# Xiugapurin/Etude

Hardware: AMD Instinct MI355X
Metric: audio-sec/s transcribed + decoder tokens/s, 3-min clip batch (higher is better)
Workload: dtype f16

## Files before the change

### etude_amd/_lib.py

```python
from __future__ import annotations

import ctypes as C
import os
from pathlib import Path

import torch

LIB_PATH = Path(os.environ["ETD_LIB_PATH"]) if os.environ.get("ETD_LIB_PATH") else Path(__file__).resolve().parent / "libetude_hip.so"

c_int_p = C.POINTER(C.c_int)
c_i32_p = C.POINTER(C.c_int32)
c_i64_p = C.POINTER(C.c_int64)
c_f32_p = C.POINTER(C.c_float)


class _SizedCfg(C.Structure):

    def __init__(self, *a, **k):
        super().__init__(*a, **k)
        self.struct_bytes = C.sizeof(type(self))


class ExtCfg(_SizedCfg):
    _fields_ = [("struct_bytes", C.c_int)] + [(n, C.c_int) for n in ("n_margin", "n_frame", "n_bin", "cnn_channel", "cnn_kernel", "hid_dim", "pf_dim",
# ... 80 lines not shown
class Job(C.Structure):
    _fields_ = [("x_ids", C.c_void_p), ("x_offsets", C.c_void_p), ("n_bars", C.c_int), ("attrs4", C.c_void_p), ("ready", C.c_void_p)]


class ScoreJob(C.Structure):
    _fields_ = [("x_ids", C.c_void_p), ("x_offsets", C.c_void_p), ("n_bars", C.c_int), ("attrs4", C.c_void_p),
                ("y_ids", C.c_void_p), ("y_offsets", C.c_void_p), ("n_y_bars", C.c_int)]


class SchedCfg(_SizedCfg):
    _fields_ = [("struct_bytes", C.c_int)] + [(n, C.c_int) for n in ("bar_bos_id", "bar_eos_id", "n_ctx_pairs", "max_position_embeddings", "max_output_tokens",
                                       "max_bar_token_limit")] + [("context_overlap_ratio", C.c_float)] + \
               [(n, C.c_int) for n in ("force_bar_tokens", "max_streams", "max_prefill_rows", "steps_per_poll")] + \
               [("temperature", C.c_float), ("top_p", C.c_float), ("seed", C.c_ulonglong), ("job_key_offset", C.c_int), ("job_key_stride", C.c_int)]


class TempoRegion(C.Structure):
    _fields_ = [("bpm", C.c_double), ("time_sig", C.c_int), ("start", C.c_double), ("downbeats", C.c_void_p), ("n_downbeats", C.c_int)]


class TokEvent(C.Structure):
    _fields_ = [("type", C.c_int32), ("value", C.c_int32)]


class Note(C.Structure):
    _fields_ = [("onset", C.c_double), ("offset", C.c_double), ("pitch", C.c_int32), ("velocity", C.c_int32)]


ABI_VERSION = 3

SIGNATURES = {
    "etd_version": (C.c_int, []),
    "etd_last_error": (C.c_char_p, []),
    "etd_build_id": (C.c_char_p, []),
    "etd_extractor_operand_type": (C.c_int, []),
    "etd_decoder_operand_type": (C.c_int, []),
    "etd_has_experiments": (C.c_int, []),
    "etd_prof_enable": (C.c_int, [C.c_int]),
    "etd_prof_reset": (C.c_int, []),
    "etd_prof_collect": (C.c_int, []),
    "etd_prof_count": (C.c_int, []),
    "etd_prof_entry": (C.c_int, [C.c_int, C.c_char_p, C.c_int, C.POINTER(C.c_double), C.POINTER(C.c_longlong),
                                 C.POINTER(C.c_double), C.POINTER(C.c_double)]),
    "etd_debug_boundary_cost": (C.c_int, [C.c_int, C.c_int, C.c_int, C.c_void_p, C.POINTER(C.c_double), C.POINTER(C.c_double)]),
    "etd_debug_linear": (C.c_int, [C.c_int, C.c_int, C.c_int, C.c_int, C.c_void_p, C.POINTER(C.c_double)]),
    "etd_debug_kernel_loop": (C.c_int, [C.c_int, C.c_int, C.c_void_p]),
    "etd_debug_g3_bounds": (C.c_int, [C.c_void_p, C.c_void_p, C.c_int, C.c_int, C.c_void_p, C.c_void_p, C.c_float, C.c_void_p, C.c_void_p]),
    "etd_debug_gemm3": (C.c_int, [C.c_void_p, C.c_int, C.c_int, C.c_void_p, C.c_void_p, C.c_int, C.c_float, C.c_int, C.c_void_p, C.c_void_p, C.c_void_p, C.c_void_p]),
    "etd_debug_gemm3_case": (C.c_int, [C.POINTER(G3Case), C.c_void_p]),
    "etd_debug_ln_rows_f32": (C.c_int, [C.c_void_p, C.c_int, C.c_int, C.c_void_p, C.c_void_p, C.c_void_p, C.c_void_p, C.c_float, C.c_void_p, C.c_void_p, C.c_void_p]),
    "etd_debug_g3_pack": (C.c_int, [C.c_void_p, C.c_int, C.c_int, C.c_void_p, C.c_longlong, C.POINTER(C.c_longlong), C.POINTER(C.c_int32)]),
    "etd_debug_attn3": (C.c_int, [C.c_void_p, C.c_void_p, C.c_void_p, C.c_void_p, C.c_int, C.c_int, C.c_int, C.c_int, C.c_float, C.c_float, C.c_float, C.c_int, C.c_void_p, C.c_void_p]),
    "etd_debug_empty_launch": (C.c_int, [C.c_int, C.c_int, C.c_int, C.c_void_p, C.c_void_p]),
    "etd_frontend_create": (C.c_int, [C.c_int, C.c_int, C.c_int, C.c_int, C.c_int, C.c_int, C.c_void_p, C.c_int, C.c_int,
                                      C.c_void_p, C.c_int, C.c_void_p, C.c_void_p, C.c_void_p, C.c_float, C.POINTER(C.c_void_p)]),
    "etd_frontend_destroy": (None, [C.c_void_p]),
    "etd_frontend_set_pad_mode": (C.c_int, [C.c_void_p, C.c_int]),
    "etd_rms_frames": (C.c_int, [C.c_void_p, C.c_longlong, C.c_int, C.c_int, C.c_void_p, C.c_longlong, C.c_void_p]),
    "etd_frontend_resampled_len": (C.c_longlong, [C.c_void_p, C.c_longlong]),
    "etd_frontend_num_frames": (C.c_longlong, [C.c_void_p, C.c_longlong]),
    "etd_frontend_run": (C.c_int, [C.c_void_p, C.c_void_p, C.c_int, C.c_longlong, C.c_void_p, C.c_void_p, C.c_longlong,
                                   C.POINTER(C.c_longlong), C.c_void_p]),
    "etd_extractor_create": (C.c_int, [C.POINTER(ExtCfg), C.POINTER(C.c_char_p), C.POINTER(C.c_void_p), c_i64_p, C.c_int,
                                       C.POINTER(C.c_void_p)]),
    "etd_extractor_destroy": (None, [C.c_void_p]),
    "etd_transcript": (C.c_int, [C.c_void_p, C.c_void_p, C.c_longlong] + [C.c_void_p] * 8 + [C.c_void_p]),
    "etd_transcript_windows": (C.c_int, [C.c_void_p, C.c_void_p, C.c_int] + [C.c_void_p] * 8 + [C.c_void_p]),
    "etd_extractor_debug_vel_logits": (C.c_int, [C.c_void_p, C.c_void_p]),
    "etd_extractor_debug_tap": (C.c_int, [C.c_void_p, C.c_int, C.c_void_p]),
    "etd_extractor_window_flops": (C.c_double, [C.c_void_p]),
    "etd_mpe2note": (C.c_int, [C.c_void_p, C.c_void_p, C.c_void_p, C.c_void_p, C.c_longlong, C.c_int, C.c_float, C.c_float,
                               C.c_float, C.c_int, C.c_int, C.c_int, C.POINTER(Note), C.c_longlong, C.POINTER(C.c_longlong)]),
    "etd_mpe2note_modes": (C.c_int, [C.c_void_p, C.c_void_p, C.c_void_p, C.c_void_p, C.c_longlong, C.c_int, C.c_float, C.c_float,
                                     C.c_float, C.c_int, C.c_int, C.c_int, C.c_int, C.c_int, C.POINTER(Note), C.c_longlong, C.POINTER(C.c_longlong)]),
    "etd_mpe2note_dev_create": (C.c_int, [C.c_int, C.POINTER(C.c_void_p)]),
    "etd_mpe2note_dev_destroy": (None, [C.c_void_p]),
    "etd_mpe2note_dev": (C.c_int, [C.c_void_p, C.c_void_p, C.c_void_p, C.c_void_p, C.c_void_p, C.c_longlong, C.c_float, C.c_float, C.c_float,
                                   C.c_int, C.c_int, C.c_int, C.POINTER(Note), C.c_longlong, C.POINTER(C.c_longlong), C.c_void_p]),
    "etd_mpe2note_dev_modes": (C.c_int, [C.c_void_p, C.c_void_p, C.c_void_p, C.c_void_p, C.c_void_p, C.c_longlong, C.c_float, C.c_float, C.c_float,
                                         C.c_int, C.c_int, C.c_int, C.c_int, C.c_int, C.POINTER(Note), C.c_longlong, C.POINTER(C.c_longlong), C.c_void_p]),
    "etd_tok_create": (C.c_int, [C.c_void_p, C.c_int, C.POINTER(C.c_void_p)]),
    "etd_tok_destroy": (None, [C.c_void_p]),
    "etd_tok_num_measures": (C.c_int, [C.c_void_p]),
    "etd_tok_measures": (C.c_int, [C.c_void_p, C.c_void_p, C.c_void_p, C.c_void_p, C.c_void_p]),
    "etd_tok_encode": (C.c_int, [C.c_void_p, C.c_void_p, C.c_longlong, C.c_int, C.c_void_p, C.c_longlong, C.POINTER(C.c_longlong)]),
    "etd_tok_split_bars": (C.c_int, [C.c_void_p, C.c_longlong, C.c_int, C.c_int, C.c_void_p, C.c_longlong, C.c_void_p, C.c_longlong,
                                     C.POINTER(C.c_longlong)]),
    "etd_tok_decode": (C.c_int, [C.c_void_p, C.c_void_p, C.c_longlong, C.c_void_p, C.c_longlong, C.c_void_p, C.c_longlong,
                                 C.POINTER(C.c_longlong)]),
    "etd_midi_write": (C.c_int, [C.c_void_p, C.c_longlong, C.c_char_p]),
    "etd_decoder_create": (C.c_int, [C.POINTER(DecCfg), C.POINTER(C.c_char_p), C.POINTER(C.c_void_p), c_i64_p, C.c_int,
                                     C.POINTER(C.c_void_p)]),
    "etd_decoder_destroy": (None, [C.c_void_p]),
    "etd_decoder_clone": (C.c_int, [C.c_void_p, C.POINTER(C.c_void_p)]),
    "etd_decoder_set_sampling": (C.c_int, [C.c_void_p, C.c_float, C.c_float, C.c_ulonglong, C.c_void_p]),
    "etd_decoder_set_keys": (C.c_int, [C.c_void_p, C.c_int, C.c_void_p, C.c_void_p]),
    "etd_decoder_begin_bar": (C.c_int, [C.c_void_p, C.c_int, C.c_void_p, C.c_void_p, C.c_void_p, C.c_int, C.c_void_p, C.c_int,
                                        C.c_int, C.c_void_p]),
    "etd_decoder_begin_bars": (C.c_int, [C.c_void_p, C.c_int] + [C.c_void_p] * 8 + [C.c_void_p]),
    "etd_decoder_step": (C.c_int, [C.c_void_p, C.c_void_p, C.c_int, C.c_int, C.c_void_p]),
    "etd_decoder_poll": (C.c_int, [C.c_void_p, C.c_void_p, C.c_int, C.c_void_p, C.c_void_p, C.c_void_p]),
    "etd_decoder_read_tokens": (C.c_int, [C.c_void_p, C.c_int, C.c_void_p, C.c_int, c_int_p, C.c_void_p]),
    "etd_decoder_read_many": (C.c_int, [C.c_void_p, C.c_int, C.c_void_p, C.c_void_p, C.c_int, C.c_void_p, C.c_void_p]),
    "etd_decoder_run_jobs": (C.c_int, [C.c_void_p, C.POINTER(SchedCfg), C.POINTER(Job), C.c_int, C.c_void_p, C.c_longlong, C.c_void_p,
                                       C.POINTER(C.c_longlong), C.c_void_p]),
    "etd_debug_assemble_prompt": (C.c_int, [C.POINTER(SchedCfg), C.c_int, C.c_void_p, C.c_void_p, C.c_void_p, C.c_void_p, C.c_void_p, C.c_void_p,
# ... 148 lines not shown
```

### etude_amd/csrc/dec_fused.hip

```cpp
#include "dec_epilogue.h"
#include "dec_kernels.h"
#include "prof.h"

#include <cstdlib>
#include <utility>
#define PM_SLOT_ELEMS (32 * 1024)

typedef const __attribute__((address_space(1))) void* pm_gptr_t;
typedef __attribute__((address_space(3))) void* pm_lptr_t;

template <int F> __device__ __forceinline__ void pm_rd(d16x8& b, unsigned addr) {
  asm volatile("ds_read_b128 %0, %1 offset:%2" : "=v"(b) : "v"(addr), "n"(F * 1024));
}
template <int F0> __device__ __forceinline__ void pm_rd4(d16x8 (&b)[4], unsigned addr) {
  pm_rd<F0>(b[0], addr); pm_rd<F0 + 1>(b[1], addr); pm_rd<F0 + 2>(b[2], addr); pm_rd<F0 + 3>(b[3], addr);
}
template <int N> __device__ __forceinline__ void pm_wait_lds() { asm volatile("s_waitcnt lgkmcnt(%0)" ::"n"(N) : "memory"); }
__device__ __forceinline__ void pm_mfma_v_a(f32x16& acc, const d16x8& af, const d16x8& bf) {
  asm volatile(ETD_MFMA16_DEC " %0, %1, %2, %0" : "+v"(acc) : "v"(af), "a"(bf));
}
template <int T, bool B_AGPR> __device__ __forceinline__ void pm_mfma_out(f32x16& acc, const d16x8& af, const d16x8& bf) {
  if constexpr (T < 8) {
    if constexpr (B_AGPR) asm volatile(ETD_MFMA16_DEC " %0, %1, %2, %0" : "+a"(acc) : "v"(af), "a"(bf));
    else                  asm volatile(ETD_MFMA16_DEC " %0, %1, %2, %0" : "+a"(acc) : "v"(af), "v"(bf));
  } else {
    if constexpr (B_AGPR) asm volatile(ETD_MFMA16_DEC " %0, %1, %2, %0" : "+v"(acc) : "v"(af), "a"(bf));
    else                  asm volatile(ETD_MFMA16_DEC " %0, %1, %2, %0" : "+v"(acc) : "v"(af), "v"(bf));
  }
}
struct PmNext { const d16* src; d16* dst; bool on; };
template <int I> __device__ __forceinline__ void pm_dma(const PmNext& n) {
  if (n.on) __builtin_amdgcn_global_load_lds((pm_gptr_t)(n.src + (I >> 2) * 2048), (pm_lptr_t)(n.dst + (I >> 2) * 2048), 16, (I & 3) * 1024, 0);
}
template <int J> struct PmMlpGroup { static constexpr int f0 = J < 8 ? 32 + 4 * J : 4 * (J - 8); };
template <int J, int JEND> __device__ __forceinline__ void pm_roll(d16x8 (&buf)[2][4], unsigned addr) {
  if constexpr (J + 1 < JEND) { pm_rd4<PmMlpGroup<J + 1>::f0>(buf[(J + 1) & 1], addr); pm_wait_lds<4>(); }
  else pm_wait_lds<0>();
}
template <int J> __device__ __forceinline__ void pm_gelu2(f32x16& acc1, const float* sbu, int kc, int h) {
#pragma unroll
  for (int e = 0; e < 2; ++e) {
    constexpr int dummy = 0; (void)dummy;
    const int i = 2 * J + e;
    acc1[i] = gelu_fast(acc1[i] + sbu[32 * kc + 8 * (i >> 2) + 4 * h + (i & 3)]);
  }
}
template <int J> __device__ __forceinline__ void pm_up_group0(d16x8 (&buf)[2][4], unsigned addr, f32x16& accn, const d16x8 (&xf)[32], const PmNext& nx) {
  pm_roll<J, 8>(buf, addr);
#pragma unroll
  for (int q = 0; q < 4; ++q) pm_mfma_v_a(accn, buf[J & 1][q], xf[4 * J + q]);
  pm_dma<2 * J>(nx); pm_dma<2 * J + 1>(nx);
  __builtin_amdgcn_sched_barrier(0);
}
template <int J, bool HALF> __device__ __forceinline__ void pm_down_group(d16x8 (&buf)[2][4], unsigned addr, f32x16 (&acc2)[16], const d16x8 (&hf)[2], const PmNext& nx) {
  pm_roll<J, 16>(buf, addr);
  constexpr int g = J - 8, t0 = 4 * (g & 3);
  pm_mfma_out<t0 + 0, false>(acc2[t0 + 0], buf[J & 1][0], hf[g >> 2]);
  pm_mfma_out<t0 + 1, false>(acc2[t0 + 1], buf[J & 1][1], hf[g >> 2]);
  pm_mfma_out<t0 + 2, false>(acc2[t0 + 2], buf[J & 1][2], hf[g >> 2]);
// ... 105 lines not shown
  if constexpr (ND >= 2) pm_dma<D0 + 1>(nx);
#undef PM_MFMA
#undef PM_PIN
  __builtin_amdgcn_sched_barrier(0);
}
template <int KS> __device__ __forceinline__ void pm_hidden_frag1(const f32x16& acc1, d16x8& hfk) {
  const d16x4 p0 = pack4d(acc1[8 * KS], acc1[8 * KS + 1], acc1[8 * KS + 2], acc1[8 * KS + 3]);
  const d16x4 p1 = pack4d(acc1[8 * KS + 4], acc1[8 * KS + 5], acc1[8 * KS + 6], acc1[8 * KS + 7]);
  const u32x2 v0 = __builtin_bit_cast(u32x2, p0), v1 = __builtin_bit_cast(u32x2, p1);
  const auto s0 = __builtin_amdgcn_permlane32_swap(v0[0], v1[0], false, false);
  const auto s1 = __builtin_amdgcn_permlane32_swap(v0[1], v1[1], false, false);
  const u32x4 o = {s0[0], s1[0], s0[1], s1[1]};
  hfk = __builtin_bit_cast(d16x8, o);
  asm volatile("s_nop 4" : "+v"(hfk) : : "memory");
}
#define PM_LOADX(dst, ptr, S) asm volatile("global_load_dwordx4 %0, %1, off offset:%2" : "=a"(dst) : "v"(ptr), "n"(32 * (S)) : "memory")
template <bool AOL>
__device__ __forceinline__ void pm_chunk(d16x8 (&buf)[2][4], unsigned sa, f32x16& prev, f32x16& cur, f32x16 (&acc2)[16], d16x8 (&xf)[32], d16x8 (&hf)[2],
                                         unsigned bias_prev, unsigned bias_cur, const PmNext& nx, const d16* ao, long long ao_off) {
  const d16* ap = nullptr;
  if constexpr (AOL) { ap = ao + ao_off; asm volatile("" : "+v"(ap)); }
#define PM_AOL(G) do { if constexpr (AOL) { PM_LOADX(xf[4 * (G)], ap, 4 * (G)); PM_LOADX(xf[4 * (G) + 1], ap, 4 * (G) + 1); PM_LOADX(xf[4 * (G) + 2], ap, 4 * (G) + 2); PM_LOADX(xf[4 * (G) + 3], ap, 4 * (G) + 3); } } while (0)
  pm_rd4<PmMlpGroup<0>::f0>(buf[0], sa);
  pm_group<0, 4, 0, 2>(buf, sa, cur, acc2, xf, hf[0], prev, bias_prev, nx);
  pm_group<1, 5, 2, 2>(buf, sa, cur, acc2, xf, hf[0], prev, bias_prev, nx);
  pm_group<2, 6, 4, 1>(buf, sa, cur, acc2, xf, hf[0], prev, bias_prev, nx);
  pm_group<3, 7, 5, 1>(buf, sa, cur, acc2, xf, hf[0], prev, bias_prev, nx);
  pm_group<4, 8, 6, 2>(buf, sa, cur, acc2, xf, hf[0], prev, bias_prev, nx);
  pm_group<5, 9, 8, 2>(buf, sa, cur, acc2, xf, hf[0], prev, bias_prev, nx);
  pm_group<6, 10, 10, 1>(buf, sa, cur, acc2, xf, hf[0], prev, bias_prev, nx);
  pm_group<7, 11, 11, 1>(buf, sa, cur, acc2, xf, hf[0], prev, bias_prev, nx);
  pm_hidden_frag1<0>(prev, hf[0]);
  pm_group<8, 12, 12, 1>(buf, sa, cur, acc2, xf, hf[0], prev, bias_prev, nx);
  PM_AOL(0);
  pm_group<9, 13, 13, 1>(buf, sa, cur, acc2, xf, hf[0], prev, bias_prev, nx);
  PM_AOL(1);
  pm_group<10, 14, 14, 1>(buf, sa, cur, acc2, xf, hf[0], prev, bias_prev, nx);
  PM_AOL(2);
  pm_group<11, 15, 15, 1>(buf, sa, cur, acc2, xf, hf[0], prev, bias_prev, nx);
  PM_AOL(3);
  pm_hidden_frag1<1>(prev, hf[1]);
  pm_group<12, 0, 0, 0>(buf, sa, cur, acc2, xf, hf[1], cur, bias_cur, nx);
  PM_AOL(4);
  pm_group<13, 1, 0, 0>(buf, sa, cur, acc2, xf, hf[1], cur, bias_cur, nx);
  PM_AOL(5);
  pm_group<14, 2, 0, 0>(buf, sa, cur, acc2, xf, hf[1], cur, bias_cur, nx);
  PM_AOL(6);
  pm_group<15, 3, 0, 0>(buf, sa, cur, acc2, xf, hf[1], cur, bias_cur, nx);
  PM_AOL(7);
#undef PM_AOL
}

#ifdef ETD_PMLP_STAMP
__device__ unsigned long long g_pmlp_stamp[64 * 4 * 8];
#define PMS(i) do { const unsigned long long t_ = __builtin_amdgcn_s_memtime(); ps_acc[i] += t_ - ps_t; ps_t = t_; } while (0)
#else
#define PMS(i) do { } while (0)
#endif
__global__ __launch_bounds__(256) __attribute__((amdgpu_waves_per_eu(1, 1))) void k_dmlp_fused(DMlpArgs a) {
  __shared__ __attribute__((aligned(16))) unsigned char smem[2 * PM_SLOT_ELEMS * 2 + 2048 * 4];
  d16* ring = reinterpret_cast<d16*>(smem);
  float* sbu = reinterpret_cast<float*>(smem + 2 * PM_SLOT_ELEMS * 2);
  const int tid = threadIdx.x, lane = tid & 63, wave = __builtin_amdgcn_readfirstlane(tid >> 6), r = lane & 31, h = lane >> 5;
  const int m = blockIdx.x * 128 + wave * 32 + r;
  const int mc = m < a.M ? m : a.M - 1;
  const unsigned ring_lds = (unsigned)reinterpret_cast<uintptr_t>(ring) + lane * 16;
#ifdef ETD_PMLP_STAMP
  const unsigned long long ps_t0 = __builtin_amdgcn_s_memtime();
#endif
  const unsigned sbu_lds = (unsigned)reinterpret_cast<uintptr_t>(sbu) + h * 16;

  auto issue = [&](int k) {
    const d16* src = a.Wm + (long long)k * PM_SLOT_ELEMS + wave * (16 * 512) + lane * 8;
    d16* dst = ring + (k & 1) * PM_SLOT_ELEMS + wave * (16 * 512);
#pragma unroll
    for (int i = 0; i < 16; ++i)
      __builtin_amdgcn_global_load_lds((pm_gptr_t)(src + i * 512), (pm_lptr_t)(dst + i * 512), 16, 0, 0);
  };
#define PM_TOP(k)                                                                                                     \
  do {                                                                                                                \
    asm volatile("s_waitcnt vmcnt(0) lgkmcnt(0)" ::: "memory");      \
    __syncthreads();                                     \
  } while (0)
  auto next_of = [&](int k) {
    return PmNext{a.Wm + (long long)(k + 1) * PM_SLOT_ELEMS + wave * (16 * 512) + lane * 8, ring + ((k + 1) & 1) * PM_SLOT_ELEMS + wave * (16 * 512), k + 1 < DMLP_NCHUNK};
  };

  issue(0);
  d16x8 xf[32];
  {
    const d16* xp = a.X2 + (long long)mc * 512 + 8 * h;
#define PM_X4(S) PM_LOADX(xf[S], xp, S); PM_LOADX(xf[(S) + 1], xp, (S) + 1); PM_LOADX(xf[(S) + 2], xp, (S) + 2); PM_LOADX(xf[(S) + 3], xp, (S) + 3)
    PM_X4(0); PM_X4(4); PM_X4(8); PM_X4(12); PM_X4(16); PM_X4(20); PM_X4(24); PM_X4(28);
#undef PM_X4
    asm volatile("s_waitcnt vmcnt(0)" ::: "memory");
  }
#ifdef ETD_PMLP_STAMP
  const unsigned long long ps_tx = __builtin_amdgcn_s_memtime();
#endif
  for (int i = tid; i < 2048; i += 256) sbu[i] = a.b_up[i];

  f32x16 acc2[16];
#pragma unroll
  for (int t = 0; t < 16; ++t)
#pragma unroll
    for (int i = 0; i < 16; ++i) acc2[t][i] = 0.f;
  f32x16 accA, accB;
  d16x8 buf[2][4], hf[2];
  using seq8 = std::make_integer_sequence<int, 8>;
  using seq16 = std::make_integer_sequence<int, 16>;
#define PM_ZERO(x) _Pragma("unroll") for (int i_ = 0; i_ < 16; ++i_) x[i_] = 0.f

  {
    PM_TOP(0);
    PM_ZERO(accA);
    pm_up_only(buf, ring_lds, accA, xf, next_of(0), seq8{});
    asm volatile("s_nop 15\n\ts_nop 15" : "+v"(accA) : : "memory");
    pm_gelu2<0>(accA, sbu, 0, h); pm_gelu2<1>(accA, sbu, 0, h);
  }
#ifdef ETD_PMLP_STAMP
  unsigned long long ps_acc[5] = {0, 0, 0, 0, 0}, ps_t = __builtin_amdgcn_s_memtime();
  const unsigned long long ps_t1 = ps_t;
#define PM_TOP_S(k)                                                                         \
  do {                                                                                      \
    if ((k) > 1) PMS(0); else ps_t = __builtin_amdgcn_s_memtime();                          \
    asm volatile("s_waitcnt vmcnt(0) lgkmcnt(0)" ::: "memory");                             \
    PMS(1);                                                                                 \
    __syncthreads();                                                                        \
    PMS(2);                                                                                 \
  } while (0)
#else
#define PM_TOP_S(k) PM_TOP(k)
#endif
#define PM_CHUNK(k, prev, cur, AOLV)                                                                                                                \
  do {                                                                                                                                          \
    PM_TOP_S(k);                                                                                                                                \
    pm_chunk<(AOLV)>(buf, ring_lds + ((k) & 1) * (PM_SLOT_ELEMS * 2), prev, cur, acc2, xf, hf, sbu_lds + ((k) - 1) * 128, sbu_lds + (k) * 128, next_of(k), a.AO, (long long)mc * a.ldao + 8 * h); \
  } while (0)
  for (int k = 1; k < 63; k += 2) {
    PM_CHUNK(k, accA, accB, false);
    PM_CHUNK(k + 1, accB, accA, false);
  }
  PM_CHUNK(63, accA, accB, true);
#ifdef ETD_PMLP_STAMP
  PMS(0);
  const unsigned long long ps_t2 = ps_t;
#endif
  {
    PM_TOP(64);
    const unsigned sa = ring_lds;
    pm_gelu2<2>(accB, sbu, 63, h); pm_gelu2<3>(accB, sbu, 63, h);
    pm_gelu2<4>(accB, sbu, 63, h); pm_gelu2<5>(accB, sbu, 63, h); pm_gelu2<6>(accB, sbu, 63, h); pm_gelu2<7>(accB, sbu, 63, h);
    pm_hidden_frags(accB, hf);
    pm_down_only(buf, sa, acc2, hf, next_of(64), seq8{});
  }
#ifdef ETD_PMLP_STAMP
  const unsigned long long ps_t2b = __builtin_amdgcn_s_memtime();
#endif
  { PM_TOP(65); pm_dense_chunk<0>(buf, ring_lds + (65 & 1) * (PM_SLOT_ELEMS * 2), acc2, xf, next_of(65), seq16{}); }
  { PM_TOP(66); pm_dense_chunk<1>(buf, ring_lds + (66 & 1) * (PM_SLOT_ELEMS * 2), acc2, xf, next_of(66), seq16{}); }
  { PM_TOP(67); pm_dense_chunk<2>(buf, ring_lds + (67 & 1) * (PM_SLOT_ELEMS * 2), acc2, xf, next_of(67), seq16{}); }
  { PM_TOP(68); pm_dense_chunk<3>(buf, ring_lds + (68 & 1) * (PM_SLOT_ELEMS * 2), acc2, xf, next_of(68), seq16{}); }
  { PM_TOP(69); pm_dense_chunk<4>(buf, ring_lds + (69 & 1) * (PM_SLOT_ELEMS * 2), acc2, xf, next_of(69), seq16{}); }
  { PM_TOP(70); pm_dense_chunk<5>(buf, ring_lds + (70 & 1) * (PM_SLOT_ELEMS * 2), acc2, xf, next_of(70), seq16{}); }
  { PM_TOP(71); pm_dense_chunk<6>(buf, ring_lds + (71 & 1) * (PM_SLOT_ELEMS * 2), acc2, xf, next_of(71), seq16{}); }
  { PM_TOP(72); pm_dense_chunk<7>(buf, ring_lds + (72 & 1) * (PM_SLOT_ELEMS * 2), acc2, xf, next_of(72), seq16{}); }

#ifdef ETD_PMLP_STAMP
  const unsigned long long ps_t3 = __builtin_amdgcn_s_memtime();
#endif
  asm volatile("s_nop 15\n\ts_nop 15" : "+a"(acc2[0]), "+a"(acc2[1]), "+a"(acc2[2]), "+a"(acc2[3]), "+a"(acc2[4]), "+a"(acc2[5]), "+a"(acc2[6]), "+a"(acc2[7]) : : "memory");
  asm volatile("" : "+v"(acc2[8]), "+v"(acc2[9]), "+v"(acc2[10]), "+v"(acc2[11]), "+v"(acc2[12]), "+v"(acc2[13]), "+v"(acc2[14]), "+v"(acc2[15]));
  __syncthreads();
  constexpr int SROW = 132;
  float* stg = reinterpret_cast<float*>(smem) + wave * (32 * SROW + 128);
  float* spar = reinterpret_cast<float*>(smem) + 4 * (32 * SROW + 128);
  for (int i = tid; i < 512; i += 256) {
    spar[i] = a.b_cat[i];
    if (a.nx1) { spar[512 + i] = a.g1[i]; spar[1024 + i] = a.b1[i]; spar[1536 + i] = a.g2[i]; spar[2048 + i] = a.b2[i]; }
  }
  __syncthreads();
  const int m0w = blockIdx.x * 128 + wave * 32;
  const int rrow = lane >> 5, rcol = lane & 31;
  f32x4 hv[16];
  auto load_rows = [&](int g) {
#pragma unroll
    for (int it = 0; it < 16; ++it) {
      int mm = m0w + 2 * it + rrow; mm = mm < a.M ? mm : a.M - 1;
      hv[it] = *reinterpret_cast<const f32x4*>(a.hin + (long long)mm * 512 + g * 128 + rcol * 4);
    }
  };
  load_rows(0);
  float gs[16][2];
#pragma unroll
  for (int g = 0; g < 4; ++g) {
#pragma unroll
    for (int it = 0; it < 16; ++it) *reinterpret_cast<f32x4*>(stg + (2 * it + rrow) * SROW + rcol * 4) = hv[it];
    if (g < 3) load_rows(g + 1);
#pragma unroll
    for (int tt = 0; tt < 4; ++tt)
#pragma unroll
      for (int u = 0; u < 2; ++u) {
        const int t = 4 * g + tt, f0 = 32 * t + 16 * u + 8 * h;
        float* sp = stg + r * SROW + 32 * tt + 16 * u + 8 * h;
        const f32x4 ba = *reinterpret_cast<const f32x4*>(spar + f0), bb = *reinterpret_cast<const f32x4*>(spar + f0 + 4);
        const f32x4 ha = *reinterpret_cast<const f32x4*>(sp), hb = *reinterpret_cast<const f32x4*>(sp + 4);
        float sm = 0.f;
#pragma unroll
        for (int j = 0; j < 4; ++j) {
          const float va = (acc2[t][8 * u + j] + ba[j]) + ha[j], vb = (acc2[t][8 * u + 4 + j] + bb[j]) + hb[j];
          acc2[t][8 * u + j] = va; acc2[t][8 * u + 4 + j] = vb;
        }
#pragma unroll
        for (int j = 0; j < 8; ++j) sm += acc2[t][8 * u + j];
        gs[t][u] = sm;
        const f32x4 oa = {acc2[t][8 * u], acc2[t][8 * u + 1], acc2[t][8 * u + 2], acc2[t][8 * u + 3]};
        const f32x4 ob = {acc2[t][8 * u + 4], acc2[t][8 * u + 5], acc2[t][8 * u + 6], acc2[t][8 * u + 7]};
        *reinterpret_cast<f32x4*>(sp) = oa;
        *reinterpret_cast<f32x4*>(sp + 4) = ob;
      }
#pragma unroll
    for (int it = 0; it < 16; ++it) {
      const int mm = m0w + 2 * it + rrow;
      const f32x4 v = *reinterpret_cast<const f32x4*>(stg + (2 * it + rrow) * SROW + rcol * 4);
      if (mm < a.M) *reinterpret_cast<f32x4*>(a.hout + (long long)mm * 512 + g * 128 + rcol * 4) = v;
    }
  }
#ifdef ETD_PMLP_STAMP
  {
    asm volatile("s_waitcnt vmcnt(0)" ::: "memory");
    const unsigned long long ps_t4 = __builtin_amdgcn_s_memtime();
    if (lane == 0 && blockIdx.x < 64) {
      unsigned long long* o = g_pmlp_stamp + (blockIdx.x * 4 + wave) * 8;
      o[0] = ps_t2b - ps_t2; o[1] = ps_tx - ps_t0; o[2] = ps_acc[1] + ps_acc[2];
      o[3] = ps_t1 - ps_t0; o[4] = ps_t2 - ps_t1; o[5] = ps_t3 - ps_t2; o[6] = ps_t4 - ps_t3;
    }
  }
#endif
  if (!a.nx1) return;
#define PM_FOLD(gsv, tot)                                                                                             \
  {                                                                                                                   \
    _Pragma("unroll") for (int w = 8; w >= 1; w >>= 1)                                                                \
      _Pragma("unroll") for (int t = 0; t < w; ++t) { gsv[t][0] += gsv[t + w][0]; gsv[t][1] += gsv[t + w][1]; }        \
    tot = gsv[0][0] + gsv[0][1];                                                                                      \
    tot += xhalf(tot);                                                                                                \
  }
  float tot;
  PM_FOLD(gs, tot);
  const float mean = tot / 512.f;
#pragma unroll
  for (int t = 0; t < 16; ++t)
#pragma unroll
    for (int u = 0; u < 2; ++u) {
      float q = 0.f;
#pragma unroll
      for (int j = 0; j < 8; ++j) { const float d0 = acc2[t][8 * u + j] - mean; q += d0 * d0; }
      gs[t][u] = q;
    }
  float qt;
  PM_FOLD(gs, qt);
  const float rstd = rsqrtf(qt / 512.f + a.eps);
  d16* stb = reinterpret_cast<d16*>(stg);
#pragma unroll
  for (int which = 0; which < 2; ++which) {
    const float* gam = spar + (which ? 1536 : 512); const float* bet = spar + (which ? 2048 : 1024);
    d16* dstp = which ? a.nx2 : a.nx1;
#pragma unroll
    for (int hh = 0; hh < 2; ++hh) {
#pragma unroll
      for (int tt = 0; tt < 8; ++tt)
#pragma unroll
        for (int u = 0; u < 2; ++u) {
          const int t = 8 * hh + tt, f0 = 32 * t + 16 * u + 8 * h;
          const f32x4 ga = *reinterpret_cast<const f32x4*>(gam + f0), gb = *reinterpret_cast<const f32x4*>(gam + f0 + 4);
          const f32x4 ba = *reinterpret_cast<const f32x4*>(bet + f0), bb = *reinterpret_cast<const f32x4*>(bet + f0 + 4);
          d16x8 o;
#pragma unroll
          for (int j = 0; j < 4; ++j) {
            o[j] = (d16)((acc2[t][8 * u + j] - mean) * rstd * ga[j] + ba[j]); o[4 + j] = (d16)((acc2[t][8 * u + 4 + j] - mean) * rstd * gb[j] + bb[j]);
          }
          *reinterpret_cast<d16x8*>(stb + r * (2 * SROW) + 32 * tt + 16 * u + 8 * h) = o;
        }
#pragma unroll
      for (int it = 0; it < 16; ++it) {
        const int mm = m0w + 2 * it + rrow;
        const u32x4 v = *reinterpret_cast<const u32x4*>(stb + (2 * it + rrow) * (2 * SROW) + rcol * 8);
        if (mm < a.M) *reinterpret_cast<u32x4*>(dstp + (long long)mm * 512 + hh * 256 + rcol * 8) = v;
      }
    }
  }
#ifdef ETD_PMLP_STAMP
  asm volatile("s_waitcnt vmcnt(0)" ::: "memory");
  if (lane == 0 && blockIdx.x < 64) g_pmlp_stamp[(blockIdx.x * 4 + wave) * 8 + 7] = __builtin_amdgcn_s_memtime() - ps_t0;
#endif
}

#ifdef ETD_PMLP_STAMP
extern "C" int etd_debug_pmlp_stamps(unsigned long long* out) {
  HIP_TRY(hipDeviceSynchronize());
  HIP_TRY(hipMemcpyFromSymbol(out, HIP_SYMBOL(g_pmlp_stamp), sizeof(unsigned long long) * 64 * 4 * 8));
  return ETD_OK;
}
#endif
int launch_dmlp_fused(const DMlpArgs& a, hipStream_t st) {
  if (a.M <= 0 || !a.X2 || !a.AO || a.ldao < 512 || (a.ldao % 8) || !a.hin || !a.hout || a.hin == a.hout || !a.Wm || !a.b_up || !a.b_cat ||
      (((uintptr_t)a.X2 | (uintptr_t)a.AO | (uintptr_t)a.Wm | (uintptr_t)a.hin | (uintptr_t)a.hout | (uintptr_t)a.nx1 | (uintptr_t)a.nx2) & 15) ||
      (a.nx1 && (!a.nx2 || !a.g1 || !a.b1 || !a.g2 || !a.b2)))
    ETD_FAIL(ETD_EINVAL, "dmlp_fused: bad arguments");
  ProfScope ps("k_dmlp_fused", st, 2.0 * a.M * 512.0 * (2048.0 * 2 + 512.0), (double)a.M * 512 * (2 + 2 + 4 + 4 + (a.nx1 ? 4 : 0)) + (double)DMLP_STREAM_ELEMS * 2);
  hipLaunchKernelGGL(k_dmlp_fused, dim3((a.M + 127) / 128), dim3(256), 0, st, a);
  HIP_TRY(hipGetLastError());
  return ETD_OK;
}

void pack_dmlp_weights(const uint16_t* Wup, const uint16_t* Wcat, uint16_t* dst) {
  auto perm = [](int r) { const int i = (r & 3) + 4 * (r >> 3), hh = (r >> 2) & 1; return 16 * (i >> 3) + 8 * hh + (i & 7); };
  const int KC = 2560;
  for (int k = 0; k < DMLP_NCHUNK; ++k)
    for (int fr = 0; fr < 64; ++fr)
      for (int l = 0; l < 64; ++l) {
        const int r = l & 31, h = l >> 5;
        uint16_t* d = dst + (((size_t)k * 64 + fr) * 64 + l) * 8;
        for (int j = 0; j < 8; ++j) d[j] = 0;
        if (k <= 64) {
          if (fr < 32) {
            if (k == 0) continue;
            const int ks = fr >> 4, t = fr & 15, feat = 32 * t + perm(r);
            for (int j = 0; j < 8; ++j) d[j] = Wcat[(size_t)feat * KC + 32 * (k - 1) + 16 * ks + 8 * h + j];
          } else {
            if (k == 64) continue;
            const int s = fr - 32;
            for (int j = 0; j < 8; ++j) d[j] = Wup[(size_t)(32 * k + r) * 512 + 16 * s + 8 * h + j];
          }
        } else {
          const int dc = k - 65, sl = fr >> 4, t = fr & 15, feat = 32 * t + perm(r), s = 4 * dc + sl;
          for (int j = 0; j < 8; ++j) d[j] = Wcat[(size_t)feat * KC + 2048 + 16 * s + 8 * h + j];
        }
      }
}
```

### etude_amd/csrc/dec_kernels.h

```cpp
#pragma once
#include "common.h"

#ifdef ETD_DEC_BF16
typedef bf16 d16; typedef bf16x8 d16x8; typedef bf16x4 d16x4; typedef bf16x2 d16x2;
#define ETD_MFMA16_DEC "v_mfma_f32_32x32x16_bf16"
#define ETD_DEC_IS_F16 0
#ifdef __HIPCC__
__device__ __forceinline__ d16x4 pack4d(float a, float b, float c, float d) { return pack4(a, b, c, d); }
#endif
#else
typedef f16 d16; typedef f16x8 d16x8; typedef f16x4 d16x4; typedef f16x2 d16x2;
#define ETD_MFMA16_DEC "v_mfma_f32_32x32x16_f16"
#define ETD_DEC_IS_F16 1
#ifdef __HIPCC__
__device__ __forceinline__ d16x4 pack4d(float a, float b, float c, float d) { return pack4h(a, b, c, d); }
#endif
#endif

#define DS_MAX_ROWS 512
#define DS_STEP_MAX_ROWS 2048

struct DecRows {
  const int* slot;
  const int* pos;
// ... 59 lines not shown
  int pair;
  float* O;
  d16* Ob; int ldob;
  float scale;
  double bytes_hint;
  const d16* dense_w;
  float* dense_out;
  float* dbg;
  unsigned long long* stamp;
  int stamp_par;
};
int launch_dattn(const DAttnArgs& a, bool kv_bf16, hipStream_t st);
struct DRowFin {
  int* cnt; int target;
  const float* P; int nslab;
  const float* bias; const float* hin; float* hout;
  const float* g1; const float* b1; const float* g2; const float* b2; float eps;
  d16* x1; d16* x2;
};
int launch_dstep_attn_down(const DAttnArgs& a, const DGemmArgs& down, const DRowFin* fin, hipStream_t st);

struct PAttnArgs {
  const d16* Q; int ldq;
  const d16* Kc; const d16* Vc;
  long long slot_stride; int max_ctx, n_heads;
  d16* O; int ldo;
  const int* seq_row0; const int* seq_len; const int* row_slot;
  int n_seq, max_len;
  float scale_log2e;
  double flops_hint;
};
int launch_pattn(const PAttnArgs& a, hipStream_t st);

struct PQkvArgs {
  const d16* X; int ldx;
  const d16* Wf;
  const float* bias;
  int M, N;
  DecRows rows;
  const float* rope_cos; const float* rope_sin;
  d16* Qb;
  d16* Kc; d16* Vc; long long slot_stride; int max_ctx, n_heads;
};
int launch_pqkv(const PQkvArgs& a, hipStream_t st);

int launch_ln_rows(const float* h, int M, int H, const float* g1, const float* b1, const float* g2, const float* b2, float eps,
                   d16* x1, d16* x2, hipStream_t st);
int launch_resid_ln_rows(const float* P, int k_splits, const float* bias, const float* add, const float* hin, float* hout, int M, int H,
                         const float* g1, const float* b1, const float* g2, const float* b2, float eps, d16* x1, d16* x2, hipStream_t st);
int launch_gather_rows(const float* src, const int* idx, int n, int H, float* out, hipStream_t st);

#define DMLP_NCHUNK 73
#define DMLP_STREAM_ELEMS (DMLP_NCHUNK * 32 * 1024)
struct DMlpArgs {
  const d16* X2;
  const d16* AO; int ldao;
  const float* hin; float* hout;
  const d16* Wm;
  const float* b_up;
  const float* b_cat;
  const float* g1; const float* b1; const float* g2; const float* b2; float eps;
  d16* nx1; d16* nx2;
  int M;
};
int launch_dmlp_fused(const DMlpArgs& a, hipStream_t st);
void pack_dmlp_weights(const uint16_t* Wup_bf16 , const uint16_t* Wcat_bf16 , uint16_t* dst );

struct DEmbedArgs {
  const int* ids; const int* cls; const int* attrs;
  const int* cur_tok; const int* tgt_attrs;
  int tgt_cls;
  DecRows rows; int M, H, n_bins;
  const int* slots; const int* len; const int* done;
  int* row_slot_out; int* row_pos_out; int* row_active_out; int* row_sp_out;
  const float* word; const float* cls_emb; const float* attr_tab;
  float* h;
};
int launch_dembed(const DEmbedArgs& a, hipStream_t st);

struct DArgmaxArgs {
  const float* logits; int ldl; int V; int M;
  DecRows rows;
  int* cur_tok; int* len; int* done; int* n_out; int* out_tok; int out_cap; const int* eos; const int* limit;
  int set_len_from_pos;
  const DSampleCfg* samp; const unsigned long long* rng_key;
};
int launch_dargmax(const DArgmaxArgs& a, hipStream_t st);
extern "C" int etd_debug_sample_rows(const float* logits_dev, int M, int V, int ld, float temperature, float top_p, unsigned long long seed,
                                     const unsigned long long* keys_dev, const unsigned* ctrs_dev, int* out_tok_dev, void* stream);
```

### include/etude_hip_debug.h

```cpp
#ifndef ETUDE_HIP_DEBUG_H
#define ETUDE_HIP_DEBUG_H
#include "etude_hip.h"

#ifdef __cplusplus
extern "C" {
#endif

int etd_debug_boundary_cost(int n_nodes, int iters, int big_args, void* stream, double* eager_us, double* graph_us);
int etd_debug_linear(int M, int N, int K, int iters, void* stream, double* us);
int etd_debug_kernel_loop(int which, int iters, void* stream);
int etd_debug_empty_launch(int gx, int gy, int gz, int* sink_dev, void* stream);

int etd_extractor_debug_vel_logits(etd_ext*, float* vel_logits_dev);
int etd_extractor_debug_tap(etd_ext*, int stage, void* dst_dev);

int etd_debug_assemble_prompt(const etd_sched_cfg* cfg, int n_hist, const int32_t* const* hx, const int32_t* hxn, const int32_t* const* hy,
                              const int32_t* hyn, const int32_t* hattrs4, const int32_t* x, int xn, const int32_t* y_attrs4,
                              int32_t* ids_out, int32_t* cls_out, int32_t* attrs4_out, int cap, int* T_out);
int etd_debug_assemble_scored(const etd_sched_cfg* cfg, int n_hist, const int32_t* const* hx, const int32_t* hxn, const int32_t* const* hy,
                              const int32_t* hyn, const int32_t* hattrs4, const int32_t* x, int xn, const int32_t* y, int yn, const int32_t* y_attrs4,
                              int32_t* ids_out, int32_t* cls_out, int32_t* attrs4_out, int32_t* labels_out, int cap, int* T_out);

int etd_debug_decoder_checksum(etd_dec*, unsigned long long* out, int cap, void* stream);
int etd_debug_decoder_kv_rowsums(etd_dec*, unsigned* out_host, long long cap, void* stream);
int etd_debug_decoder_trace_begin(etd_dec*, int cap_steps, void* stream);
int etd_debug_decoder_trace_slabs(etd_dec*, float* out_host, long long cap_floats, int n_active, void* stream);
int etd_debug_decoder_trace_lanes(etd_dec*, float* out_host, long long cap_floats, int n_active, void* stream);
int etd_debug_decoder_trace_q(etd_dec*, float* out_host, long long cap_floats, int n_active, void* stream);
int etd_debug_decoder_peek_kv(etd_dec*, int layer, int slot, int head, int n_pos, unsigned short* k_out, unsigned short* v_out, void* stream);
int etd_debug_decoder_trace_read(etd_dec*, unsigned* out_host, long long cap_words, int n_active, int* steps_done, void* stream);

int etd_debug_decoder_force_pair(etd_dec*, int mode);
int etd_debug_decoder_step_logits(etd_dec*, int on, float* out_host, int n_active, void* stream);
int etd_debug_decoder_bar_logits(etd_dec*, float* out_host, int n, void* stream);
typedef struct etd_debug_dec_taps {
  int struct_bytes;
  unsigned layer_mask;
  int rows, hidden, intermediate, slab_cap;
  int slices;
  float* hin;
  void *ln1, *ln2;
  float* q;
  void* qb;
  void* xcat;
  float* slabs;
  float* hout;
  int32_t *step_slot, *step_pos;
  float* next_h; void *next_ln1, *next_ln2; int32_t* next_pos;
} etd_debug_dec_taps;
int etd_debug_decoder_stage_taps(etd_dec*, const etd_debug_dec_taps* taps, void* stream);
int etd_debug_decoder_peek_kv_many(etd_dec*, int layer, int n, const int32_t* slots, int n_pos, unsigned short* k_out, unsigned short* v_out, void* stream);

int etd_debug_sample_rows(const float* logits_dev, int M, int V, int ld, float temperature, float top_p, unsigned long long seed,
                          const unsigned long long* keys_dev, const unsigned* ctrs_dev, int* out_tok_dev, void* stream);

int etd_debug_gemm3(const float* x_dev, int M, int K, const float* w_host, const float* bias_host, int N, float x_bound, int gelu, float* y_dev,
                    const float* ln_g_host, const float* ln_b_host, void* stream);
enum { ETD_G3_KERNEL_AUTO = 0 , ETD_G3_KERNEL_TILE = 1 , ETD_G3_KERNEL_SMALL = 2  };
enum { ETD_G3_EPI_BIAS = 0, ETD_G3_EPI_GELU = 1, ETD_G3_EPI_RESID = 2, ETD_G3_EPI_LOGITS = 3, ETD_G3_EPI_QKV = 4, ETD_G3_EPI_RELU = 6 };
typedef struct etd_debug_g3_case {
  int struct_bytes;
  int kernel, epi;
  int M, N, K, ldx, ldy;
  const float* X; long long x_elems;
// ... 53 lines not shown
```

Baseline: 582.9.

## Make fused decoder MLP kernel persistent with weight-stream prefetch across row blocks

The fused decoder MLP kernel now launches at most one workgroup per CU. Each workgroup loops over row blocks with a grid stride. While finishing one block it prefetches the first weight chunk and the next block's activations, using a parity-swapped, gap-padded LDS ring so the epilogue staging does not clobber the in-flight slot. It also moves the bias and layer-norm parameter loads into LDS once, ahead of the loop. The aim is to avoid relaunching and re-priming the weight stream per 128-row block and to overlap the tail of one block with the start of the next. The cost is more LDS use, more complex indexing, and possible load imbalance when the block count is not a multiple of the CU count.

```diff
diff --git a/etude_amd/_lib.py b/etude_amd/_lib.py
--- a/etude_amd/_lib.py
+++ b/etude_amd/_lib.py
@@ -156,6 +156,7 @@
     "etd_debug_g3_pack": (C.c_int, [C.c_void_p, C.c_int, C.c_int, C.c_void_p, C.c_longlong, C.POINTER(C.c_longlong), C.POINTER(C.c_int32)]),
     "etd_debug_attn3": (C.c_int, [C.c_void_p, C.c_void_p, C.c_void_p, C.c_void_p, C.c_int, C.c_int, C.c_int, C.c_int, C.c_float, C.c_float, C.c_float, C.c_int, C.c_void_p, C.c_void_p]),
     "etd_debug_empty_launch": (C.c_int, [C.c_int, C.c_int, C.c_int, C.c_void_p, C.c_void_p]),
+    "etd_debug_dmlp_walk": (C.c_int, [C.c_int, C.c_int, c_int_p, c_int_p, c_int_p, C.c_void_p, C.c_void_p, C.c_void_p, C.c_int]),
     "etd_frontend_create": (C.c_int, [C.c_int, C.c_int, C.c_int, C.c_int, C.c_int, C.c_int, C.c_void_p, C.c_int, C.c_int,
                                       C.c_void_p, C.c_int, C.c_void_p, C.c_void_p, C.c_void_p, C.c_float, C.POINTER(C.c_void_p)]),
     "etd_frontend_destroy": (None, [C.c_void_p]),
diff --git a/etude_amd/csrc/dec_fused.hip b/etude_amd/csrc/dec_fused.hip
--- a/etude_amd/csrc/dec_fused.hip
+++ b/etude_amd/csrc/dec_fused.hip
@@ -5,6 +5,8 @@
 #include <cstdlib>
 #include <utility>
 #define PM_SLOT_ELEMS (32 * 1024)
+#define PM_GAP_ELEMS (2 * 1024)
+#define PM_SLOT_PITCH (PM_SLOT_ELEMS + PM_GAP_ELEMS)
 
 typedef const __attribute__((address_space(1))) void* pm_gptr_t;
 typedef __attribute__((address_space(3))) void* pm_lptr_t;
@@ -216,53 +218,68 @@
 }
 
 #ifdef ETD_PMLP_STAMP
-__device__ unsigned long long g_pmlp_stamp[64 * 4 * 8];
+__device__ unsigned long long g_pmlp_stamp[2 * 64 * 4 * 8];
 #define PMS(i) do { const unsigned long long t_ = __builtin_amdgcn_s_memtime(); ps_acc[i] += t_ - ps_t; ps_t = t_; } while (0)
 #else
 #define PMS(i) do { } while (0)
 #endif
 __global__ __launch_bounds__(256) __attribute__((amdgpu_waves_per_eu(1, 1))) void k_dmlp_fused(DMlpArgs a) {
-  __shared__ __attribute__((aligned(16))) unsigned char smem[2 * PM_SLOT_ELEMS * 2 + 2048 * 4];
+  __shared__ __attribute__((aligned(16))) unsigned char smem[(PM_SLOT_PITCH + PM_SLOT_ELEMS) * 2 + 2048 * 4 + 2560 * 4];
   d16* ring = reinterpret_cast<d16*>(smem);
-  float* sbu = reinterpret_cast<float*>(smem + 2 * PM_SLOT_ELEMS * 2);
-  const int tid = threadIdx.x, lane = tid & 63, wave = __builtin_amdgcn_readfirstlane(tid >> 6), r = lane & 31, h = lane >> 5;
-  const int m = blockIdx.x * 128 + wave * 32 + r;
-  const int mc = m < a.M ? m : a.M - 1;
-  const unsigned ring_lds = (unsigned)reinterpret_cast<uintptr_t>(ring) + lane * 16;
-#ifdef ETD_PMLP_STAMP
-  const unsigned long long ps_t0 = __builtin_amdgcn_s_memtime();
-#endif
-  const unsigned sbu_lds = (unsigned)reinterpret_cast<uintptr_t>(sbu) + h * 16;
-
-  auto issue = [&](int k) {
-    const d16* src = a.Wm + (long long)k * PM_SLOT_ELEMS + wave * (16 * 512) + lane * 8;
-    d16* dst = ring + (k & 1) * PM_SLOT_ELEMS + wave * (16 * 512);
-#pragma unroll
-    for (int i = 0; i < 16; ++i)
-      __builtin_amdgcn_global_load_lds((pm_gptr_t)(src + i * 512), (pm_lptr_t)(dst + i * 512), 16, 0, 0);
-  };
+  float* sbu = reinterpret_cast<float*>(smem + (PM_SLOT_PITCH + PM_SLOT_ELEMS) * 2);
+  float* spar = sbu + 2048;
+  const int tid = threadIdx.x, wave = __builtin_amdgcn_readfirstlane(tid >> 6);
+  const int nblk = dmlp_blocks(a.M);
+
+  int par = 0;
+#define PM_SLOT_LDS(k) (ring_lds + (unsigned)((((k) & 1) ^ par) * (PM_SLOT_PITCH * 2)))
 #define PM_TOP(k)                                                                                                     \
   do {                                                                                                                \
     asm volatile("s_waitcnt vmcnt(0) lgkmcnt(0)" ::: "memory");      \
     __syncthreads();                                     \
   } while (0)
-  auto next_of = [&](int k) {
-    return PmNext{a.Wm + (long long)(k + 1) * PM_SLOT_ELEMS + wave * (16 * 512) + lane * 8, ring + ((k + 1) & 1) * PM_SLOT_ELEMS + wave * (16 * 512), k + 1 < DMLP_NCHUNK};
+
+  int b = blockIdx.x;
+#ifdef ETD_PMLP_STAMP
+  unsigned long long ps_t0 = __builtin_amdgcn_s_memtime();
+#endif
+  {
+    const d16* src = a.Wm + wave * (16 * 512) + (tid & 63) * 8;
+    d16* dst = ring + wave * (16 * 512);
+#pragma unroll
+    for (int i = 0; i < 16; ++i)
+      __builtin_amdgcn_global_load_lds((pm_gptr_t)(src + i * 512), (pm_lptr_t)(dst + i * 512), 16, 0, 0);
+  }
+  d16x8 xf[32];
+#define PM_X4(S) PM_LOADX(xf[S], xp, S); PM_LOADX(xf[(S) + 1], xp, (S) + 1); PM_LOADX(xf[(S) + 2], xp, (S) + 2); PM_LOADX(xf[(S) + 3], xp, (S) + 3)
+  {
+    const int m = b * DMLP_BLOCK_ROWS + wave * 32 + (tid & 31);
+    const d16* xp = a.X2 + (long long)(m < a.M ? m : a.M - 1) * 512 + 8 * ((tid >> 5) & 1);
+    PM_X4(0); PM_X4(4); PM_X4(8); PM_X4(12); PM_X4(16); PM_X4(20); PM_X4(24); PM_X4(28);
+  }
+  for (int i = tid; i < 2048; i += 256) sbu[i] = a.b_up[i];
+  for (int i = tid; i < 512; i += 256) {
+    spar[i] = a.b_cat[i];
+    if (a.nx1) { spar[512 + i] = a.g1[i]; spar[1024 + i] = a.b1[i]; spar[1536 + i] = a.g2[i]; spar[2048 + i] = a.b2[i]; }
+  }
+
+  for (;;) {
+  int lane = tid & 63;
+  asm volatile("" : "+v"(lane));
+  const int r = lane & 31, h = lane >> 5;
+  const unsigned ring_lds = (unsigned)reinterpret_cast<uintptr_t>(ring) + lane * 16;
+  const unsigned sbu_lds = (unsigned)reinterpret_cast<uintptr_t>(sbu) + h * 16;
+  auto next_of = [&](int k, bool more) {
+    const int kn = k + 1 < DMLP_NCHUNK ? k + 1 : 0;
+    return PmNext{a.Wm + (long long)kn * PM_SLOT_ELEMS + wave * (16 * 512) + lane * 8, ring + (((k + 1) & 1) ^ par) * PM_SLOT_PITCH + wave * (16 * 512), k + 1 < DMLP_NCHUNK || more};
   };
-
-  issue(0);
-  d16x8 xf[32];
-  {
-    const d16* xp = a.X2 + (long long)mc * 512 + 8 * h;
-#define PM_X4(S) PM_LOADX(xf[S], xp, S); PM_LOADX(xf[(S) + 1], xp, (S) + 1); PM_LOADX(xf[(S) + 2], xp, (S) + 2); PM_LOADX(xf[(S) + 3], xp, (S) + 3)
-    PM_X4(0); PM_X4(4); PM_X4(8); PM_X4(12); PM_X4(16); PM_X4(20); PM_X4(24); PM_X4(28);
-#undef PM_X4
-    asm volatile("s_waitcnt vmcnt(0)" ::: "memory");
-  }
-#ifdef ETD_PMLP_STAMP
+  const int mc = [&] { const int m = b * DMLP_BLOCK_ROWS + wave * 32 + r; return m < a.M ? m : a.M - 1; }();
+  const int bn = dmlp_next_block(b, (int)gridDim.x);
+  const bool more = bn < nblk;
+#ifdef ETD_PMLP_STAMP
+  asm volatile("s_waitcnt vmcnt(0)" ::: "memory");
   const unsigned long long ps_tx = __builtin_amdgcn_s_memtime();
 #endif
-  for (int i = tid; i < 2048; i += 256) sbu[i] = a.b_up[i];
 
   f32x16 acc2[16];
 #pragma unroll
@@ -273,12 +290,14 @@
   d16x8 buf[2][4], hf[2];
   using seq8 = std::make_integer_sequence<int, 8>;
   using seq16 = std::make_integer_sequence<int, 16>;
-#define PM_ZERO(x) _Pragma("unroll") for (int i_ = 0; i_ < 16; ++i_) x[i_] = 0.f
+  float zero_ = 0.f;
+  asm volatile("" : "+v"(zero_));
+#define PM_ZERO(x) _Pragma("unroll") for (int i_ = 0; i_ < 16; ++i_) x[i_] = zero_
 
   {
     PM_TOP(0);
     PM_ZERO(accA);
-    pm_up_only(buf, ring_lds, accA, xf, next_of(0), seq8{});
+    pm_up_only(buf, PM_SLOT_LDS(0), accA, xf, next_of(0, more), seq8{});
     asm volatile("s_nop 15\n\ts_nop 15" : "+v"(accA) : : "memory");
     pm_gelu2<0>(accA, sbu, 0, h); pm_gelu2<1>(accA, sbu, 0, h);
   }
@@ -299,7 +318,7 @@
 #define PM_CHUNK(k, prev, cur, AOLV)                                                                                                                \
   do {                                                                                                                                          \
     PM_TOP_S(k);                                                                                                                                \
-    pm_chunk<(AOLV)>(buf, ring_lds + ((k) & 1) * (PM_SLOT_ELEMS * 2), prev, cur, acc2, xf, hf, sbu_lds + ((k) - 1) * 128, sbu_lds + (k) * 128, next_of(k), a.AO, (long long)mc * a.ldao + 8 * h); \
+    pm_chunk<(AOLV)>(buf, PM_SLOT_LDS(k), prev, cur, acc2, xf, hf, sbu_lds + ((k) - 1) * 128, sbu_lds + (k) * 128, next_of(k, more), a.AO, (long long)mc * a.ldao + 8 * h); \
   } while (0)
   for (int k = 1; k < 63; k += 2) {
     PM_CHUNK(k, accA, accB, false);
@@ -312,23 +331,23 @@
 #endif
   {
     PM_TOP(64);
-    const unsigned sa = ring_lds;
+    const unsigned sa = PM_SLOT_LDS(64);
     pm_gelu2<2>(accB, sbu, 63, h); pm_gelu2<3>(accB, sbu, 63, h);
     pm_gelu2<4>(accB, sbu, 63, h); pm_gelu2<5>(accB, sbu, 63, h); pm_gelu2<6>(accB, sbu, 63, h); pm_gelu2<7>(accB, sbu, 63, h);
     pm_hidden_frags(accB, hf);
-    pm_down_only(buf, sa, acc2, hf, next_of(64), seq8{});
+    pm_down_only(buf, sa, acc2, hf, next_of(64, more), seq8{});
   }
 #ifdef ETD_PMLP_STAMP
   const unsigned long long ps_t2b = __builtin_amdgcn_s_memtime();
 #endif
-  { PM_TOP(65); pm_dense_chunk<0>(buf, ring_lds + (65 & 1) * (PM_SLOT_ELEMS * 2), acc2, xf, next_of(65), seq16{}); }
-  { PM_TOP(66); pm_dense_chunk<1>(buf, ring_lds + (66 & 1) * (PM_SLOT_ELEMS * 2), acc2, xf, next_of(66), seq16{}); }
-  { PM_TOP(67); pm_dense_chunk<2>(buf, ring_lds + (67 & 1) * (PM_SLOT_ELEMS * 2), acc2, xf, next_of(67), seq16{}); }
-  { PM_TOP(68); pm_dense_chunk<3>(buf, ring_lds + (68 & 1) * (PM_SLOT_ELEMS * 2), acc2, xf, next_of(68), seq16{}); }
-  { PM_TOP(69); pm_dense_chunk<4>(buf, ring_lds + (69 & 1) * (PM_SLOT_ELEMS * 2), acc2, xf, next_of(69), seq16{}); }
-  { PM_TOP(70); pm_dense_chunk<5>(buf, ring_lds + (70 & 1) * (PM_SLOT_ELEMS * 2), acc2, xf, next_of(70), seq16{}); }
-  { PM_TOP(71); pm_dense_chunk<6>(buf, ring_lds + (71 & 1) * (PM_SLOT_ELEMS * 2), acc2, xf, next_of(71), seq16{}); }
-  { PM_TOP(72); pm_dense_chunk<7>(buf, ring_lds + (72 & 1) * (PM_SLOT_ELEMS * 2), acc2, xf, next_of(72), seq16{}); }
+  { PM_TOP(65); pm_dense_chunk<0>(buf, PM_SLOT_LDS(65), acc2, xf, next_of(65, more), seq16{}); }
+  { PM_TOP(66); pm_dense_chunk<1>(buf, PM_SLOT_LDS(66), acc2, xf, next_of(66, more), seq16{}); }
+  { PM_TOP(67); pm_dense_chunk<2>(buf, PM_SLOT_LDS(67), acc2, xf, next_of(67, more), seq16{}); }
+  { PM_TOP(68); pm_dense_chunk<3>(buf, PM_SLOT_LDS(68), acc2, xf, next_of(68, more), seq16{}); }
+  { PM_TOP(69); pm_dense_chunk<4>(buf, PM_SLOT_LDS(69), acc2, xf, next_of(69, more), seq16{}); }
+  { PM_TOP(70); pm_dense_chunk<5>(buf, PM_SLOT_LDS(70), acc2, xf, next_of(70, more), seq16{}); }
+  { PM_TOP(71); pm_dense_chunk<6>(buf, PM_SLOT_LDS(71), acc2, xf, next_of(71, more), seq16{}); }
+  { PM_TOP(72); pm_dense_chunk<7>(buf, PM_SLOT_LDS(72), acc2, xf, next_of(72, more), seq16{}); }
 
 #ifdef ETD_PMLP_STAMP
   const unsigned long long ps_t3 = __builtin_amdgcn_s_memtime();
@@ -337,14 +356,8 @@
   asm volatile("" : "+v"(acc2[8]), "+v"(acc2[9]), "+v"(acc2[10]), "+v"(acc2[11]), "+v"(acc2[12]), "+v"(acc2[13]), "+v"(acc2[14]), "+v"(acc2[15]));
   __syncthreads();
   constexpr int SROW = 132;
-  float* stg = reinterpret_cast<float*>(smem) + wave * (32 * SROW + 128);
-  float* spar = reinterpret_cast<float*>(smem) + 4 * (32 * SROW + 128);
-  for (int i = tid; i < 512; i += 256) {
-    spar[i] = a.b_cat[i];
-    if (a.nx1) { spar[512 + i] = a.g1[i]; spar[1024 + i] = a.b1[i]; spar[1536 + i] = a.g2[i]; spar[2048 + i] = a.b2[i]; }
-  }
-  __syncthreads();
-  const int m0w = blockIdx.x * 128 + wave * 32;
+  float* stg = reinterpret_cast<float*>(smem) + par * (PM_SLOT_ELEMS / 2) + wave * (32 * SROW + 128);
+  const int m0w = b * DMLP_BLOCK_ROWS + wave * 32;
   const int rrow = lane >> 5, rcol = lane & 31;
   f32x4 hv[16];
   auto load_rows = [&](int g) {
@@ -394,14 +407,14 @@
   {
     asm volatile("s_waitcnt vmcnt(0)" ::: "memory");
     const unsigned long long ps_t4 = __builtin_amdgcn_s_memtime();
-    if (lane == 0 && blockIdx.x < 64) {
-      unsigned long long* o = g_pmlp_stamp + (blockIdx.x * 4 + wave) * 8;
+    if (lane == 0 && blockIdx.x < 64 && b < 2 * (int)gridDim.x) {
+      unsigned long long* o = g_pmlp_stamp + ((b / (int)gridDim.x * 64 + blockIdx.x) * 4 + wave) * 8;
       o[0] = ps_t2b - ps_t2; o[1] = ps_tx - ps_t0; o[2] = ps_acc[1] + ps_acc[2];
       o[3] = ps_t1 - ps_t0; o[4] = ps_t2 - ps_t1; o[5] = ps_t3 - ps_t2; o[6] = ps_t4 - ps_t3;
     }
   }
 #endif
-  if (!a.nx1) return;
+  if (a.nx1) {
 #define PM_FOLD(gsv, tot)                                                                                             \
   {                                                                                                                   \
     _Pragma("unroll") for (int w = 8; w >= 1; w >>= 1)                                                                \
@@ -453,26 +466,53 @@
       }
     }
   }
-#ifdef ETD_PMLP_STAMP
-  asm volatile("s_waitcnt vmcnt(0)" ::: "memory");
-  if (lane == 0 && blockIdx.x < 64) g_pmlp_stamp[(blockIdx.x * 4 + wave) * 8 + 7] = __builtin_amdgcn_s_memtime() - ps_t0;
-#endif
+  }
+    if (!more) break;
+  {
+    const int m = bn * DMLP_BLOCK_ROWS + wave * 32 + r;
+    const d16* xp = a.X2 + (long long)(m < a.M ? m : a.M - 1) * 512 + 8 * h;
+    PM_X4(0); PM_X4(4); PM_X4(8); PM_X4(12); PM_X4(16); PM_X4(20); PM_X4(24); PM_X4(28);
+  }
+#ifdef ETD_PMLP_STAMP
+  {
+    asm volatile("s_waitcnt vmcnt(0)" ::: "memory");
+    const unsigned long long t_ = __builtin_amdgcn_s_memtime();
+    if (lane == 0 && blockIdx.x < 64 && b < 2 * (int)gridDim.x) g_pmlp_stamp[((b / (int)gridDim.x * 64 + blockIdx.x) * 4 + wave) * 8 + 7] = t_ - ps_t0;
+    ps_t0 = t_;
+  }
+#endif
+    b = bn; par ^= 1;
+  }
+#undef PM_X4
 }
 
 #ifdef ETD_PMLP_STAMP
 extern "C" int etd_debug_pmlp_stamps(unsigned long long* out) {
   HIP_TRY(hipDeviceSynchronize());
-  HIP_TRY(hipMemcpyFromSymbol(out, HIP_SYMBOL(g_pmlp_stamp), sizeof(unsigned long long) * 64 * 4 * 8));
+  HIP_TRY(hipMemcpyFromSymbol(out, HIP_SYMBOL(g_pmlp_stamp), sizeof(unsigned long long) * 2 * 64 * 4 * 8));
   return ETD_OK;
 }
 #endif
+extern "C" int etd_debug_dmlp_walk(int M, int cus, int* block_rows, int* blocks, int* grid, int* visits, int* owner, int* rows, int cap) {
+  if (M <= 0 || cus <= 0 || !block_rows || !blocks || !grid || !visits || !owner || !rows) ETD_FAIL(ETD_EINVAL, "dmlp_walk: bad arguments");
+  const int nb = dmlp_blocks(M), g = dmlp_grid(M, cus);
+  *block_rows = DMLP_BLOCK_ROWS; *blocks = nb; *grid = g;
+  if (cap < nb) ETD_FAIL(ETD_ENOMEM, "dmlp_walk: %d blocks, room for %d", nb, cap);
+  for (int i = 0; i < nb; ++i) { visits[i] = 0; owner[i] = -1; rows[i] = 0; }
+  for (int wg = 0; wg < g; ++wg)
+    for (int b = wg; b < nb; b = dmlp_next_block(b, g)) { ++visits[b]; owner[b] = wg; rows[b] = dmlp_block_rows(M, b); }
+  return ETD_OK;
+}
 int launch_dmlp_fused(const DMlpArgs& a, hipStream_t st) {
   if (a.M <= 0 || !a.X2 || !a.AO || a.ldao < 512 || (a.ldao % 8) || !a.hin || !a.hout || a.hin == a.hout || !a.Wm || !a.b_up || !a.b_cat ||
       (((uintptr_t)a.X2 | (uintptr_t)a.AO | (uintptr_t)a.Wm | (uintptr_t)a.hin | (uintptr_t)a.hout | (uintptr_t)a.nx1 | (uintptr_t)a.nx2) & 15) ||
       (a.nx1 && (!a.nx2 || !a.g1 || !a.b1 || !a.g2 || !a.b2)))
     ETD_FAIL(ETD_EINVAL, "dmlp_fused: bad arguments");
   ProfScope ps("k_dmlp_fused", st, 2.0 * a.M * 512.0 * (2048.0 * 2 + 512.0), (double)a.M * 512 * (2 + 2 + 4 + 4 + (a.nx1 ? 4 : 0)) + (double)DMLP_STREAM_ELEMS * 2);
-  hipLaunchKernelGGL(k_dmlp_fused, dim3((a.M + 127) / 128), dim3(256), 0, st, a);
+  int dev = 0, cus = 0;
+  HIP_TRY(hipGetDevice(&dev));
+  HIP_TRY(hipDeviceGetAttribute(&cus, hipDeviceAttributeMultiprocessorCount, dev));
+  hipLaunchKernelGGL(k_dmlp_fused, dim3(dmlp_grid(a.M, cus)), dim3(256), 0, st, a);
   HIP_TRY(hipGetLastError());
   return ETD_OK;
 }
diff --git a/etude_amd/csrc/dec_kernels.h b/etude_amd/csrc/dec_kernels.h
--- a/etude_amd/csrc/dec_kernels.h
+++ b/etude_amd/csrc/dec_kernels.h
@@ -135,6 +135,11 @@
 
 #define DMLP_NCHUNK 73
 #define DMLP_STREAM_ELEMS (DMLP_NCHUNK * 32 * 1024)
+#define DMLP_BLOCK_ROWS 128
+__host__ __device__ inline int dmlp_blocks(int M) { return (M + DMLP_BLOCK_ROWS - 1) / DMLP_BLOCK_ROWS; }
+__host__ __device__ inline int dmlp_grid(int M, int cus) { const int nb = dmlp_blocks(M); return nb < cus ? nb : (cus > 0 ? cus : 1); }
+__host__ __device__ inline int dmlp_next_block(int b, int grid) { return b + grid; }
+__host__ __device__ inline int dmlp_block_rows(int M, int b) { const int left = M - b * DMLP_BLOCK_ROWS; return left < DMLP_BLOCK_ROWS ? left : DMLP_BLOCK_ROWS; }
 struct DMlpArgs {
   const d16* X2;
   const d16* AO; int ldao;
diff --git a/include/etude_hip_debug.h b/include/etude_hip_debug.h
--- a/include/etude_hip_debug.h
+++ b/include/etude_hip_debug.h
@@ -10,6 +10,8 @@
 int etd_debug_linear(int M, int N, int K, int iters, void* stream, double* us);
 int etd_debug_kernel_loop(int which, int iters, void* stream);
 int etd_debug_empty_launch(int gx, int gy, int gz, int* sink_dev, void* stream);
+
+int etd_debug_dmlp_walk(int M, int cus, int* block_rows, int* blocks, int* grid, int* visits, int* owner, int* rows, int cap);
 
 int etd_extractor_debug_vel_logits(etd_ext*, float* vel_logits_dev);
 int etd_extractor_debug_tap(etd_ext*, int stage, void* dst_dev);
```

Result: no change. 584.5 (median of 2 runs) (+0.3%).
